# PaddlePaddle/PARL

Measured on NVIDIA H100. Metric: env_steps_per_sec_impala_4096_actors, higher is better.
Workload: dtype bf16 network (fp32 accumulate, fp32 master weights) / f32 scans+losses

## Files before the change

### parl_b200/csrc/shiftconv.cu

```cuda
#include <cuda_bf16.h>

#include "common.cuh"
#include "tma.cuh"
#include "u8win.cuh"
#include "wgmma.cuh"

namespace rl {

constexpr int kScBM = 128;
constexpr int kScMaxStages = 8;
constexpr int kScThreads = 384;

struct ShiftConvArgs {
  const float* bias;
  __nv_bfloat16* out;
  int H, W, KH, KW, Hout, Wout;
  int Q;
  int wrows;
  int num_tiles, relu;
  int stages;
  int out_mode;
  int OGH, OGW;
  int row_shift;
  int flip;
  const __nv_bfloat16* mask;
  float in_scale;
};

__device__ __forceinline__ uint32_t s_pack_bf16x2(float lo, float hi) {
  uint32_t d;
  asm("cvt.rn.bf16x2.f32 %0, %1, %2;\n" : "=r"(d) : "f"(hi), "f"(lo));
  return d;
}
__device__ __forceinline__ uint32_t s_pack_relu_bf16x2(float lo, float hi) {
  uint32_t d;
  asm("cvt.rn.relu.bf16x2.f32 %0, %1, %2;\n" : "=r"(d) : "f"(hi), "f"(lo));
  return d;
}

template <int COUT, int CBLK, int KS, int MODE, bool U8IN = false>
__global__ void __launch_bounds__(U8IN ? kScThreads + kU8Threads : kScThreads, 1)
    shiftconv_fwd_kernel(const __grid_constant__ CUtensorMap map_in, const __grid_constant__ CUtensorMap map_w,
                         const ShiftConvArgs g) {
  static_assert(!U8IN || CBLK == 1, "the uint8 window is one 64-channel block");
  constexpr int W_KB = COUT * 128;
  extern __shared__ __align__(1024) unsigned char smem_dyn[];
  unsigned char* smem = smem_dyn + ((1024u - (smem_u32(smem_dyn) & 1023u)) & 1023u);
  constexpr int num_kb = KS * KS * CBLK;
  const int win_bytes = (g.wrows * 128 + 1023) & ~1023;
  unsigned char* sW = smem;
  unsigned char* sWin = smem + ((num_kb * W_KB + 1023) & ~1023);
  __shared__ __align__(8) unsigned long long full_bar[kScMaxStages], empty_bar[kScMaxStages], w_bar;
  __shared__ __align__(8) unsigned long long u8_full[kU8Stages], u8_empty[kU8Stages];
  const uint32_t nstages = (uint32_t)g.stages;
  unsigned char* sStage = sWin + nstages * CBLK * win_bytes;

  const int warp = threadIdx.x >> 5, lane = threadIdx.x & 31;
  if (threadIdx.x == 0) {
    tma_prefetch_desc(&map_in);
    tma_prefetch_desc(&map_w);
    for (int s = 0; s < kScMaxStages; ++s) {
      mbar_init(&full_bar[s], U8IN ? kU8Threads : 1);
      mbar_init(&empty_bar[s], 1);
    }
    for (int s = 0; s < kU8Stages; ++s) {
      mbar_init(&u8_full[s], 1);
      mbar_init(&u8_empty[s], kU8Threads);
    }
    mbar_init(&w_bar, 1);
    fence_mbar_init();
  }
  __syncthreads();
  if (threadIdx.x == 128) {
    mbar_arrive_expect_tx(&w_bar, (uint32_t)(num_kb * W_KB));
    for (int kb = 0; kb < num_kb; ++kb) tma_load_2d(sW + kb * W_KB, &map_w, kb * 64, 0, &w_bar);
  }
  pdl_wait();
  pdl_trigger();

  if (warp < 4) {
    if (warp == 0 && lane == 0) {
      uint32_t s = 0, par = 1;
      if (U8IN) {
        const int sbytes = u8_stage_bytes(g.wrows);
        for (int tile = blockIdx.x; tile < g.num_tiles; tile += gridDim.x) {
          mbar_wait(&u8_empty[s], par);
          mbar_arrive_expect_tx(&u8_full[s], (uint32_t)(g.wrows * 64));
          tma_load_2d(sStage + s * sbytes, &map_in, 0, tile * kScBM + g.row_shift, &u8_full[s]);
          if (++s == kU8Stages) s = 0, par ^= 1u;
        }
      } else {
        for (int tile = blockIdx.x; tile < g.num_tiles; tile += gridDim.x) {
          mbar_wait(&empty_bar[s], par);
          mbar_arrive_expect_tx(&full_bar[s], (uint32_t)(CBLK * g.wrows * 128));
#pragma unroll
          for (int cb = 0; cb < CBLK; ++cb)
            tma_load_2d(sWin + (s * CBLK + cb) * win_bytes, &map_in, cb * 64, tile * kScBM + g.row_shift, &full_bar[s]);
          if (++s == nstages) s = 0, par ^= 1u;
        }
      }
    }
    return;
  }
  if (U8IN && threadIdx.x >= kScThreads) {
    const int ct = threadIdx.x - kScThreads;
    const int sbytes = u8_stage_bytes(g.wrows);
    const float bias = -8388608.0f * g.in_scale;
    uint32_t s = 0, epar = 1, ss = 0, fpar = 0;
    for (int tile = blockIdx.x; tile < g.num_tiles; tile += gridDim.x) {
      mbar_wait(&u8_full[ss], fpar);
      mbar_wait(&empty_bar[s], epar);
      u8_window_to_bf16_sw128(sStage + ss * sbytes, sWin + s * win_bytes, g.wrows, ct, g.in_scale, bias);
      fence_proxy_async_smem();
      mbar_arrive(&full_bar[s]);
      mbar_arrive(&u8_empty[ss]);
      if (++s == nstages) s = 0, epar ^= 1u;
      if (++ss == kU8Stages) ss = 0, fpar ^= 1u;
    }
    return;
  }
  const int c = (threadIdx.x >> 7) - 1, t = threadIdx.x & 127;
  mbar_wait(&w_bar, 0);
  uint32_t tap_off[KS * KS];
#pragma unroll
  for (int r = 0; r < KS; ++r)
#pragma unroll
    for (int sx = 0; sx < KS; ++sx)
      tap_off[r * KS + sx] = (uint32_t)(g.flip ? (KS - 1 - r) * g.W + (KS - 1 - sx) : r * g.W + sx) * 8u;
  const uint32_t w_lo = gmma_lo(sW), win_lo0 = gmma_lo(sWin);
  const uint32_t win16 = (uint32_t)win_bytes >> 4;
  float bias_r[MODE == 0 ? COUT / 2 : 1];
  if (MODE == 0) {
#pragma unroll
    for (int i = 0; i < COUT / 2; ++i) bias_r[i] = __ldg(g.bias + gmma_col(t, i));
  }
  const bool relu = g.relu != 0;
  const bool has_mask = MODE == 1 && g.mask != nullptr;
  const int HW = g.H * g.W;
  uint32_t s = (uint32_t)c, full_par = 0;
  for (long long tile = blockIdx.x + (long long)c * gridDim.x; tile < g.num_tiles; tile += 2 * gridDim.x) {
    float d[2][COUT / 2];
    mbar_wait(&full_bar[s], full_par);
    wgmma_fence();
    const uint32_t a_lo = win_lo0 + s * (CBLK * win16);
#pragma unroll
    for (int h = 0; h < 2; ++h) {
#pragma unroll
      for (int tap = 0; tap < KS * KS; ++tap) {
#pragma unroll
        for (int cb = 0; cb < CBLK; ++cb) {
#pragma unroll
          for (int k = 0; k < 4; ++k)
            wgmma_bf16<COUT>(d[h], gmma_desc(kGmmaHiSw128, a_lo + h * 512u + cb * win16 + tap_off[tap] + 2u * k),
                             gmma_desc(kGmmaHiSw128, w_lo + (uint32_t)((tap * CBLK + cb) * (W_KB >> 4) + 2 * k)),
                             (tap | cb | k) != 0 ? 1u : 0u);
        }
      }
    }
    wgmma_commit();
    wgmma_wait<0>();
    wgmma_fence_regs(d[0]);
    wgmma_fence_regs(d[1]);
    if (t == 0) mbar_arrive(&empty_bar[s]);
    s += 2;
    if (s >= nstages) s -= nstages, full_par ^= 1u;
#pragma unroll
    for (int h = 0; h < 2; ++h) {
#pragma unroll
      for (int rr = 0; rr < 2; ++rr) {
        const int q = (int)tile * kScBM + 64 * h + gmma_row(t, 2 * rr);
        const int n = q / HW;
        const int rem = q - n * HW;
        const int y = rem / g.W, x = rem - y * g.W;
        const bool valid = q < g.Q && y < g.Hout && x < g.Wout;
        size_t obase = 0;
        if (g.out_mode == 0) {
          obase = ((size_t)(n * g.OGH + y) * g.OGW + x) * COUT;
        } else if (g.out_mode == 1) {
          const int yp = y + 2, xp = x + 2;
          obase = (((size_t)n * 12 + (yp >> 1)) * 12 + (xp >> 1)) * (4 * COUT) + (size_t)(((yp & 1) * 2 + (xp & 1)) * COUT);
        }
        constexpr int MJ = COUT <= 64 ? COUT / 8 : (KS == 2 ? 4 : 2);
#pragma unroll
        for (int j0 = 0; j0 < COUT / 8; j0 += MJ) {
        uint32_t mw[MJ];
        if (has_mask && q < g.Q) {
#pragma unroll
          for (int jj = 0; jj < MJ; ++jj)
            mw[jj] = __ldg(reinterpret_cast<const unsigned int*>(g.mask + (size_t)q * COUT + gmma_col(t, 4 * (j0 + jj) + 2 * rr)));
        }
#pragma unroll
        for (int jj = 0; jj < MJ; ++jj) {
          const int j = j0 + jj, i = 4 * j + 2 * rr, col = gmma_col(t, i);
          bool ok = valid;
          size_t dst_off = obase + col;
          if (g.out_mode == 2) {
            const int blk = col >> 5, py = 2 * y + (blk >> 1) - 2, px = 2 * x + (blk & 1) - 2;
            ok = q < g.Q && py >= 0 && py < 20 && px >= 0 && px < 20;
            dst_off = (((size_t)n * 21 + py) * 21 + px) * 32 + (col & 31);
          }
          if (!ok) continue;
          uint32_t pk;
          if (MODE == 0) {
            const float v0 = d[h][i] + bias_r[i], v1 = d[h][i + 1] + bias_r[i + 1];
            pk = relu ? s_pack_relu_bf16x2(v0, v1) : s_pack_bf16x2(v0, v1);
          } else {
            pk = s_pack_bf16x2(d[h][i], d[h][i + 1]);
            if (has_mask) {
              pk &= __hgt2_mask(*reinterpret_cast<const __nv_bfloat162*>(&mw[jj]), __floats2bfloat162_rn(0.f, 0.f));
            }
          }
          *reinterpret_cast<uint32_t*>(g.out + dst_off) = pk;
        }
        }
      }
    }
  }
}

template <int COUT, int CBLK, int KS, int MODE, bool U8IN = false>
__global__ void __launch_bounds__(U8IN ? kScThreads + kU8Threads : kScThreads, 1)
    shiftconv_coltap_kernel(const __grid_constant__ CUtensorMap map_in, const __grid_constant__ CUtensorMap map_w,
                            const ShiftConvArgs g) {
  static_assert(!U8IN || CBLK == 1, "the uint8 window is one 64-channel block");
  constexpr int W_KB = COUT * 128;
  constexpr int ST = kScBM - (KS - 1);
  extern __shared__ __align__(1024) unsigned char smem_dyn[];
  unsigned char* smem = smem_dyn + ((1024u - (smem_u32(smem_dyn) & 1023u)) & 1023u);
  constexpr int num_kb = KS * KS * CBLK;
  const int win_bytes = (g.wrows * 128 + 1023) & ~1023;
  unsigned char* sW = smem;
  unsigned char* sWin = smem + ((num_kb * W_KB + 1023) & ~1023);
  __shared__ __align__(8) unsigned long long full_bar[kScMaxStages], empty_bar[kScMaxStages], w_bar;
  __shared__ __align__(8) unsigned long long u8_full[kU8Stages], u8_empty[kU8Stages];
  const uint32_t nstages = (uint32_t)g.stages;
  unsigned char* sStage = sWin + nstages * CBLK * win_bytes;
  float* sAcc = reinterpret_cast<float*>(sStage + (U8IN ? kU8Stages * u8_stage_bytes(g.wrows) : 0));

  const int warp = threadIdx.x >> 5, lane = threadIdx.x & 31;
  if (threadIdx.x == 0) {
    tma_prefetch_desc(&map_in);
    tma_prefetch_desc(&map_w);
    for (int s = 0; s < kScMaxStages; ++s) {
      mbar_init(&full_bar[s], U8IN ? kU8Threads : 1);
      mbar_init(&empty_bar[s], 1);
    }
    for (int s = 0; s < kU8Stages; ++s) {
      mbar_init(&u8_full[s], 1);
      mbar_init(&u8_empty[s], kU8Threads);
    }
    mbar_init(&w_bar, 1);
    fence_mbar_init();
  }
  __syncthreads();
  if (threadIdx.x == 128) {
    mbar_arrive_expect_tx(&w_bar, (uint32_t)(num_kb * W_KB));
    for (int kb = 0; kb < num_kb; ++kb) tma_load_2d(sW + kb * W_KB, &map_w, kb * 64, 0, &w_bar);
  }
  pdl_wait();
  pdl_trigger();

  if (warp < 4) {
    if (warp == 0 && lane == 0) {
      uint32_t s = 0, par = 1;
      if (U8IN) {
        const int sbytes = u8_stage_bytes(g.wrows);
        for (int tile = blockIdx.x; tile < g.num_tiles; tile += gridDim.x) {
          mbar_wait(&u8_empty[s], par);
          mbar_arrive_expect_tx(&u8_full[s], (uint32_t)(g.wrows * 64));
          tma_load_2d(sStage + s * sbytes, &map_in, 0, tile * ST + g.row_shift, &u8_full[s]);
          if (++s == kU8Stages) s = 0, par ^= 1u;
        }
      } else {
        for (int tile = blockIdx.x; tile < g.num_tiles; tile += gridDim.x) {
          mbar_wait(&empty_bar[s], par);
          mbar_arrive_expect_tx(&full_bar[s], (uint32_t)(CBLK * g.wrows * 128));
#pragma unroll
          for (int cb = 0; cb < CBLK; ++cb)
            tma_load_2d(sWin + (s * CBLK + cb) * win_bytes, &map_in, cb * 64, tile * ST + g.row_shift, &full_bar[s]);
          if (++s == nstages) s = 0, par ^= 1u;
        }
      }
    }
    return;
  }
  if (U8IN && threadIdx.x >= kScThreads) {
    const int ct = threadIdx.x - kScThreads;
    const int sbytes = u8_stage_bytes(g.wrows);
    const float bias = -8388608.0f * g.in_scale;
    uint32_t s = 0, epar = 1, ss = 0, fpar = 0;
    for (int tile = blockIdx.x; tile < g.num_tiles; tile += gridDim.x) {
      mbar_wait(&u8_full[ss], fpar);
      mbar_wait(&empty_bar[s], epar);
      u8_window_to_bf16_sw128(sStage + ss * sbytes, sWin + s * win_bytes, g.wrows, ct, g.in_scale, bias);
      fence_proxy_async_smem();
      mbar_arrive(&full_bar[s]);
      mbar_arrive(&u8_empty[ss]);
      if (++s == nstages) s = 0, epar ^= 1u;
      if (++ss == kU8Stages) ss = 0, fpar ^= 1u;
    }
    return;
  }
  const int c = (threadIdx.x >> 7) - 1, t = threadIdx.x & 127;
  mbar_wait(&w_bar, 0);
  uint32_t row_off[KS];
#pragma unroll
  for (int r = 0; r < KS; ++r) row_off[r] = (uint32_t)((g.flip ? KS - 1 - r : r) * g.W) * 8u;
  const uint32_t w_lo = gmma_lo(sW), win_lo0 = gmma_lo(sWin);
  const uint32_t win16 = (uint32_t)win_bytes >> 4;
  float bias_r[MODE == 0 ? COUT / 2 : 1];
  if (MODE == 0) {
#pragma unroll
    for (int i = 0; i < COUT / 2; ++i) bias_r[i] = __ldg(g.bias + gmma_col(t, i));
  }
  const bool relu = g.relu != 0;
  const bool has_mask = MODE == 1 && g.mask != nullptr;
  const int HW = g.H * g.W;
  uint32_t s = 0, full_par = 0;
  for (int tile = blockIdx.x; tile < g.num_tiles; tile += gridDim.x) {
    mbar_wait(&full_bar[s], full_par);
    const uint32_t a_lo = win_lo0 + s * (CBLK * win16) + (uint32_t)c * 512u;
#pragma unroll
    for (int sh = 0; sh < KS; ++sh) {
      const int sc = g.flip ? KS - 1 - sh : sh;
      float d[COUT / 2];
      wgmma_fence();
#pragma unroll
      for (int r = 0; r < KS; ++r)
#pragma unroll
        for (int cb = 0; cb < CBLK; ++cb)
#pragma unroll
          for (int k = 0; k < 4; ++k)
            wgmma_bf16<COUT>(d, gmma_desc(kGmmaHiSw128, a_lo + cb * win16 + row_off[r] + 2u * k),
                             gmma_desc(kGmmaHiSw128, w_lo + (uint32_t)(((r * KS + sc) * CBLK + cb) * (W_KB >> 4) + 2 * k)),
                             (r | cb | k) != 0 ? 1u : 0u);
      wgmma_commit();
      wgmma_wait<0>();
      wgmma_fence_regs(d);
      named_bar_sync(1, 256);
      if (sh == KS - 1 && threadIdx.x == 128) mbar_arrive(&empty_bar[s]);
#pragma unroll
      for (int i = 0; i < COUT / 2; i += 2) {
        const int p = 64 * c + gmma_row(t, i) - sh;
        if (p < 0) continue;
        float2* cell = reinterpret_cast<float2*>(sAcc + p * COUT + gmma_col(t, i));
        if (sh == 0) {
          *cell = make_float2(d[i], d[i + 1]);
        } else {
          const float2 o = *cell;
          *cell = make_float2(o.x + d[i], o.y + d[i + 1]);
        }
      }
    }
    if (++s == nstages) s = 0, full_par ^= 1u;
    named_bar_sync(1, 256);
#pragma unroll
    for (int i = 0; i < COUT / 2; i += 2) {
      const int p = 64 * c + gmma_row(t, i), col = gmma_col(t, i);
      const int q = tile * ST + p;
      if (p >= ST || q >= g.Q) continue;
      const float2 v = *reinterpret_cast<const float2*>(sAcc + p * COUT + col);
      const int n = q / HW;
      const int rem = q - n * HW;
      const int y = rem / g.W, x = rem - y * g.W;
      bool ok = y < g.Hout && x < g.Wout;
      size_t dst_off;
      if (g.out_mode == 0) {
        dst_off = ((size_t)(n * g.OGH + y) * g.OGW + x) * COUT + col;
      } else if (g.out_mode == 1) {
        const int yp = y + 2, xp = x + 2;
        dst_off = (((size_t)n * 12 + (yp >> 1)) * 12 + (xp >> 1)) * (4 * COUT) + (size_t)(((yp & 1) * 2 + (xp & 1)) * COUT) + col;
      } else {
        const int blk = col >> 5, py = 2 * y + (blk >> 1) - 2, px = 2 * x + (blk & 1) - 2;
        ok = py >= 0 && py < 20 && px >= 0 && px < 20;
        dst_off = (((size_t)n * 21 + py) * 21 + px) * 32 + (col & 31);
      }
      if (!ok) continue;
      uint32_t pk;
      if (MODE == 0) {
        const float v0 = v.x + bias_r[i], v1 = v.y + bias_r[i + 1];
        pk = relu ? s_pack_relu_bf16x2(v0, v1) : s_pack_bf16x2(v0, v1);
      } else {
        pk = s_pack_bf16x2(v.x, v.y);
        if (has_mask) {
          const uint32_t mw = __ldg(reinterpret_cast<const unsigned int*>(g.mask + (size_t)q * COUT + col));
          pk &= __hgt2_mask(*reinterpret_cast<const __nv_bfloat162*>(&mw), __floats2bfloat162_rn(0.f, 0.f));
        }
      }
      *reinterpret_cast<uint32_t*>(g.out + dst_off) = pk;
    }
  }
}

static int sc_make_map(CUtensorMap* map, const void* base, uint64_t cols, uint64_t rows, uint32_t box_rows) {
  typedef CUresult (*EncodeFn)(CUtensorMap*, CUtensorMapDataType, cuuint32_t, void*, const cuuint64_t*, const cuuint64_t*,
                               const cuuint32_t*, const cuuint32_t*, CUtensorMapInterleave, CUtensorMapSwizzle,
                               CUtensorMapL2promotion, CUtensorMapFloatOOBfill);
  static EncodeFn fn = nullptr;
  if (!fn) {
    void* p = nullptr;
    cudaDriverEntryPointQueryResult q;
    if (cudaGetDriverEntryPoint("cuTensorMapEncodeTiled", &p, cudaEnableDefault, &q) != cudaSuccess || !p) return -1;
    fn = reinterpret_cast<EncodeFn>(p);
  }
  const cuuint64_t gdim[2] = {cols, rows};
  const cuuint64_t gstride[1] = {cols * 2};
  const cuuint32_t box[2] = {64, box_rows};
  const cuuint32_t estr[2] = {1, 1};
  return fn(map, CU_TENSOR_MAP_DATA_TYPE_BFLOAT16, 2, const_cast<void*>(base), gdim, gstride, box, estr,
            CU_TENSOR_MAP_INTERLEAVE_NONE, CU_TENSOR_MAP_SWIZZLE_128B, CU_TENSOR_MAP_L2_PROMOTION_L2_128B,
            CU_TENSOR_MAP_FLOAT_OOB_FILL_NONE) == CUDA_SUCCESS
             ? 0
             : -2;
}

static size_t u8_ring_bytes(int wrows) { return (size_t)kU8Stages * (size_t)((wrows * 64 + 1023) & ~1023); }

template <int COUT, int CBLK, int KS, int MODE, bool U8IN = false>
static void launch_shiftconv(const CUtensorMap& mi, const CUtensorMap& mw, const ShiftConvArgs& g, int num_kb, int sms,
                             cudaStream_t st) {
  const size_t win = (size_t)((g.wrows * 128 + 1023) & ~1023);
  const size_t smem = (size_t)((num_kb * COUT * 128 + 1023) & ~1023) + (size_t)g.stages * CBLK * win + 1024 +
                      (U8IN ? u8_ring_bytes(g.wrows) : 0);
  auto kern = shiftconv_fwd_kernel<COUT, CBLK, KS, MODE, U8IN>;
  RL_SMEM_OPTIN(kern);
  const int grid = g.num_tiles < sms ? g.num_tiles : sms;
  launch_chain(kern, dim3(grid), dim3(U8IN ? kScThreads + kU8Threads : kScThreads), smem, st, mi, mw, g);
}

template <int COUT, int CBLK, int KS, int MODE, bool U8IN = false>
static void launch_coltap(const CUtensorMap& mi, const CUtensorMap& mw, const ShiftConvArgs& g, int num_kb, int sms,
                          cudaStream_t st) {
  const size_t win = (size_t)((g.wrows * 128 + 1023) & ~1023);
  const size_t smem = (size_t)((num_kb * COUT * 128 + 1023) & ~1023) + (size_t)g.stages * CBLK * win + 1024 +
                      (U8IN ? u8_ring_bytes(g.wrows) : 0) + (size_t)kScBM * COUT * sizeof(float);
  auto kern = shiftconv_coltap_kernel<COUT, CBLK, KS, MODE, U8IN>;
  RL_SMEM_OPTIN(kern);
  const int grid = g.num_tiles < sms ? g.num_tiles : sms;
  launch_chain(kern, dim3(grid), dim3(U8IN ? kScThreads + kU8Threads : kScThreads), smem, st, mi, mw, g);
}

}

using namespace rl;

static int g_sc_form = 0;
extern "C" int rl_debug_set_shiftconv_form(int form) {
  RL_CHECK_ARG(form == 0 || form == 1, "shiftconv form must be 0 (per-tap) or 1 (column taps)");
  g_sc_form = form;
  return RL_OK;
}

extern "C" int rl_debug_set_shiftconv_base_offset(int enable) {
  RL_CHECK_ARG(enable == 0, "shiftconv base_offset must be 0 (the swizzle phase comes from the shared-memory address)");
  return RL_OK;
}

static int shiftconv_launch(const void* in, const void* weight, const float* bias, void* out, int N, int H, int W,
                            int Cin, int Cout, int KH, int KW, int relu, int out_mode, int Hout, int Wout, int OGH, int OGW,
                            int transposed, const void* mask, rl_stream_t stream, const char* name, int u8in = 0,
                            float in_scale = 1.f) {
  RL_CHECK_ARG(in && weight && out && N > 0, "%s: bad argument", name);
  RL_CHECK_ARG(aligned16(in) && aligned16(weight) && aligned16(out) && (!mask || aligned16(mask)),
               "%s: 16-byte alignment required", name);
  RL_CHECK_ARG((Cout == 32 || Cout == 64 || Cout == 128) && (Cin == 64 || Cin == 128),
               "%s: Cin in {64,128}, Cout in {32,64,128}", name);
  RL_CHECK_ARG(KH == KW && (KH == 2 || KH == 3) && KH <= H && KW <= W, "%s: filter must be 2x2 or 3x3", name);
  ShiftConvArgs g;
  g.bias = bias, g.out = (__nv_bfloat16*)out, g.H = H, g.W = W, g.KH = KH, g.KW = KW;
  g.Hout = Hout, g.Wout = Wout, g.OGH = OGH, g.OGW = OGW;
  const long long Q = (long long)N * H * W;
  RL_CHECK_ARG(Q < (1LL << 31), "%s: too many positions", name);
  const int coltap = g_sc_form == 1;
  const int tile_rows = coltap ? kScBM - (KW - 1) : kScBM;
  g.Q = (int)Q, g.wrows = kScBM + (KH - 1) * W + (coltap ? 0 : KW - 1), g.relu = relu, g.out_mode = out_mode;
  g.row_shift = transposed ? -((KH - 1) * W + (KW - 1)) : 0, g.flip = transposed;
  g.mask = (const __nv_bfloat16*)mask, g.in_scale = in_scale;
  RL_CHECK_ARG(g.wrows <= 256, "%s: window of %d rows exceeds the TMA box limit", name, g.wrows);
  g.num_tiles = (int)((Q + tile_rows - 1) / tile_rows);
  const int cblk = Cin / 64, num_kb = KH * KW * cblk;
  const size_t win = (size_t)((g.wrows * 128 + 1023) & ~1023);
  {
    const size_t acc = coltap ? (size_t)kScBM * Cout * sizeof(float) : 0;
    const size_t budget = 220 * 1024 - ((size_t)num_kb * Cout * 128 + 2048) - (u8in ? u8_ring_bytes(g.wrows) : 0) - acc;
    long long st = (long long)(budget / ((size_t)cblk * win));
    if (st > kScMaxStages) st = kScMaxStages;
    if (mask && st > 4) st = 4;
    RL_CHECK_ARG(st >= 2, "%s: weights + windows do not fit in shared memory", name);
    g.stages = (int)st;
  }
  alignas(64) CUtensorMap mi, mw;
  if ((u8in ? make_tensor_map_u8_rows64(&mi, in, (uint64_t)Q, (uint32_t)g.wrows)
            : sc_make_map(&mi, in, (uint64_t)Cin, (uint64_t)Q, (uint32_t)g.wrows)) ||
      sc_make_map(&mw, weight, (uint64_t)KH * KW * Cin, (uint64_t)Cout, (uint32_t)Cout)) {
    set_error("%s: cuTensorMapEncodeTiled failed", name);
    return RL_ERR_CUDA;
  }
  int dev = 0, sms = 132;
  cudaGetDevice(&dev);
  cudaDeviceGetAttribute(&sms, cudaDevAttrMultiProcessorCount, dev);
  sms = effective_sms(sms);
  cudaStream_t st = (cudaStream_t)stream;
  const int key = (u8in ? 1000000 : 0) + (transposed ? 100000 : 0) + Cout * 100 + cblk * 10 + KH;
  if (coltap) {
    switch (key) {
      case 1003212: launch_coltap<32, 1, 2, 0, true>(mi, mw, g, num_kb, sms, st); break;
      case 3212: launch_coltap<32, 1, 2, 0>(mi, mw, g, num_kb, sms, st); break;
      case 6422: launch_coltap<64, 2, 2, 0>(mi, mw, g, num_kb, sms, st); break;
      case 6413: launch_coltap<64, 1, 3, 0>(mi, mw, g, num_kb, sms, st); break;
      case 6412: launch_coltap<64, 1, 2, 0>(mi, mw, g, num_kb, sms, st); break;
      case 6423: launch_coltap<64, 2, 3, 0>(mi, mw, g, num_kb, sms, st); break;
      case 106413: launch_coltap<64, 1, 3, 1>(mi, mw, g, num_kb, sms, st); break;
      case 112812: launch_coltap<128, 1, 2, 1>(mi, mw, g, num_kb, sms, st); break;
      case 106412: launch_coltap<64, 1, 2, 1>(mi, mw, g, num_kb, sms, st); break;
      case 112813: launch_coltap<128, 1, 3, 1>(mi, mw, g, num_kb, sms, st); break;
      default:
        set_error("%s: no instantiation for Cout=%d Cin=%d %dx%d", name, Cout, Cin, KH, KW);
        return RL_ERR_BAD_ARG;
    }
  } else
  switch (key) {
    case 1003212: launch_shiftconv<32, 1, 2, 0, true>(mi, mw, g, num_kb, sms, st); break;
    case 3212: launch_shiftconv<32, 1, 2, 0>(mi, mw, g, num_kb, sms, st); break;
    case 6422: launch_shiftconv<64, 2, 2, 0>(mi, mw, g, num_kb, sms, st); break;
    case 6413: launch_shiftconv<64, 1, 3, 0>(mi, mw, g, num_kb, sms, st); break;
    case 6412: launch_shiftconv<64, 1, 2, 0>(mi, mw, g, num_kb, sms, st); break;
    case 6423: launch_shiftconv<64, 2, 3, 0>(mi, mw, g, num_kb, sms, st); break;
    case 106413: launch_shiftconv<64, 1, 3, 1>(mi, mw, g, num_kb, sms, st); break;
    case 112812: launch_shiftconv<128, 1, 2, 1>(mi, mw, g, num_kb, sms, st); break;
    case 106412: launch_shiftconv<64, 1, 2, 1>(mi, mw, g, num_kb, sms, st); break;
    case 112813: launch_shiftconv<128, 1, 3, 1>(mi, mw, g, num_kb, sms, st); break;
    default:
      set_error("%s: no instantiation for Cout=%d Cin=%d %dx%d", name, Cout, Cin, KH, KW);
      return RL_ERR_BAD_ARG;
  }
  cudaError_t e = cudaGetLastError();
  if (e != cudaSuccess) {
    set_error("%s: launch failed: %s", name, cudaGetErrorString(e));
    return RL_ERR_CUDA;
  }
  return RL_OK;
}

extern "C" int rl_conv2d_s1_nhwc_bf16_fwd(const void* in, const void* weight_krsc, const float* bias, void* out, int N,
                                          int H, int W, int Cin, int Cout, int KH, int KW, int relu, int out_mode,
                                          rl_stream_t stream) {
  RL_CHECK_ARG(bias, "conv2d_s1: bias required");
  RL_CHECK_ARG(out_mode == 0 || (out_mode == 1 && H - KH + 1 == 20 && W - KW + 1 == 20),
               "conv2d_s1: out_mode 1 is the 20x20 -> [12,12,4*Cout] layout");
  return shiftconv_launch(in, weight_krsc, bias, out, N, H, W, Cin, Cout, KH, KW, relu, out_mode, H - KH + 1, W - KW + 1,
                          H - KH + 1, W - KW + 1, 0, nullptr, stream, "conv2d_s1");
}

extern "C" int rl_conv2d_s1_u8in_bf16_fwd(const void* in_u8, float in_scale, const void* weight_krsc, const float* bias,
                                          void* out, int N, int H, int W, int Cout, int KH, int KW, int relu,
                                          int out_mode, rl_stream_t stream) {
  RL_CHECK_ARG(bias, "conv2d_s1_u8in: bias required");
  RL_CHECK_ARG(Cout == 32 && KH == 2 && KW == 2, "conv2d_s1_u8in: built for the 2x2, 64 -> 32 layer (conv1, space-to-depth)");
  RL_CHECK_ARG(out_mode == 0 || (out_mode == 1 && H - KH + 1 == 20 && W - KW + 1 == 20),
               "conv2d_s1_u8in: out_mode 1 is the 20x20 -> [12,12,4*Cout] layout");
  return shiftconv_launch(in_u8, weight_krsc, bias, out, N, H, W, 64, Cout, KH, KW, relu, out_mode, H - KH + 1,
                          W - KW + 1, H - KH + 1, W - KW + 1, 0, nullptr, stream, "conv2d_s1_u8in", 1, in_scale);
}

extern "C" int rl_conv2d_s1_nhwc_bf16_dgrad(const void* dout_grid, const void* weight_t_krsc, const void* act_mask,
                                            void* din, int N, int H, int W, int Cout, int Cin, int KH, int KW,
                                            int out_mode, int OGH, int OGW, rl_stream_t stream) {
  RL_CHECK_ARG(out_mode == 0 || (out_mode == 2 && H == 12 && W == 12 && Cin == 128),
               "conv2d_s1_dgrad: out_mode 2 is the [12,12,128] -> [21,21,32] layout");
  return shiftconv_launch(dout_grid, weight_t_krsc, nullptr, din, N, H, W, Cout, Cin, KH, KW, 0, out_mode, H, W,
                          out_mode == 0 ? OGH : 0, out_mode == 0 ? OGW : 0, 1, act_mask, stream, "conv2d_s1_dgrad");
}
```

### parl_b200/csrc/wgmma.cuh

```cuda
#pragma once
#include <stdint.h>

#include "tma.cuh"

namespace rl {

#ifdef __CUDACC__
constexpr uint32_t kGmmaHiSw128 = (uint32_t)(1024 >> 4) | (1u << 30);
constexpr uint32_t kGmmaHiSw64 = (uint32_t)(512 >> 4) | (2u << 30);
constexpr uint32_t kGmmaLoLbo1 = 1u << 16;
__device__ __forceinline__ uint64_t gmma_desc(uint32_t hi, uint32_t lo) { return ((uint64_t)hi << 32) | (uint64_t)lo; }
__device__ __forceinline__ uint32_t gmma_lo(const void* smem) { return (smem_u32(smem) >> 4) + kGmmaLoLbo1; }

__device__ __forceinline__ void wgmma_fence() { asm volatile("wgmma.fence.sync.aligned;\n" ::: "memory"); }
__device__ __forceinline__ void wgmma_commit() { asm volatile("wgmma.commit_group.sync.aligned;\n" ::: "memory"); }
template <int N>
__device__ __forceinline__ void wgmma_wait() {
  asm volatile("wgmma.wait_group.sync.aligned %0;\n" ::"n"(N) : "memory");
}
template <int R>
__device__ __forceinline__ void wgmma_fence_regs(float (&d)[R]) {
#pragma unroll
  for (int i = 0; i < R; ++i) asm volatile("" : "+f"(d[i])::"memory");
}
__device__ __forceinline__ void named_bar_sync(int id, int nthreads) {
  asm volatile("bar.sync %0, %1;\n" ::"r"(id), "r"(nthreads) : "memory");
}

template <int TA, int TB>
__device__ __forceinline__ void wgmma_bf16_n32(float (&d)[16], uint64_t da, uint64_t db, uint32_t acc) {
  asm volatile(
      "{\n.reg .pred p;\nsetp.ne.b32 p, %18, 0;\n"
      "wgmma.mma_async.sync.aligned.m64n32k16.f32.bf16.bf16 {%0, %1, %2, %3, %4, %5, %6, %7, %8, %9, %10, %11, %12, %13, %14, %15}, %16, %17, p, 1, 1, %19, %20;\n}\n"
      : "+f"(d[0]), "+f"(d[1]), "+f"(d[2]), "+f"(d[3]), "+f"(d[4]), "+f"(d[5]), "+f"(d[6]), "+f"(d[7]), "+f"(d[8]), "+f"(d[9]), "+f"(d[10]), "+f"(d[11]), "+f"(d[12]), "+f"(d[13]), "+f"(d[14]), "+f"(d[15])
      : "l"(da), "l"(db), "r"(acc), "n"(TA), "n"(TB));
}
template <int TA, int TB>
__device__ __forceinline__ void wgmma_bf16_n64(float (&d)[32], uint64_t da, uint64_t db, uint32_t acc) {
  asm volatile(
      "{\n.reg .pred p;\nsetp.ne.b32 p, %34, 0;\n"
      "wgmma.mma_async.sync.aligned.m64n64k16.f32.bf16.bf16 {%0, %1, %2, %3, %4, %5, %6, %7, %8, %9, %10, %11, %12, %13, %14, %15, %16, %17, %18, %19, %20, %21, %22, %23, %24, %25, %26, %27, %28, %29, %30, %31}, %32, %33, p, 1, 1, %35, %36;\n}\n"
      : "+f"(d[0]), "+f"(d[1]), "+f"(d[2]), "+f"(d[3]), "+f"(d[4]), "+f"(d[5]), "+f"(d[6]), "+f"(d[7]), "+f"(d[8]), "+f"(d[9]), "+f"(d[10]), "+f"(d[11]), "+f"(d[12]), "+f"(d[13]), "+f"(d[14]), "+f"(d[15]), "+f"(d[16]), "+f"(d[17]), "+f"(d[18]), "+f"(d[19]), "+f"(d[20]), "+f"(d[21]), "+f"(d[22]), "+f"(d[23]), "+f"(d[24]), "+f"(d[25]), "+f"(d[26]), "+f"(d[27]), "+f"(d[28]), "+f"(d[29]), "+f"(d[30]), "+f"(d[31])
      : "l"(da), "l"(db), "r"(acc), "n"(TA), "n"(TB));
}
template <int TA, int TB>
__device__ __forceinline__ void wgmma_bf16_n128(float (&d)[64], uint64_t da, uint64_t db, uint32_t acc) {
  asm volatile(
      "{\n.reg .pred p;\nsetp.ne.b32 p, %66, 0;\n"
      "wgmma.mma_async.sync.aligned.m64n128k16.f32.bf16.bf16 {%0, %1, %2, %3, %4, %5, %6, %7, %8, %9, %10, %11, %12, %13, %14, %15, %16, %17, %18, %19, %20, %21, %22, %23, %24, %25, %26, %27, %28, %29, %30, %31, %32, %33, %34, %35, %36, %37, %38, %39, %40, %41, %42, %43, %44, %45, %46, %47, %48, %49, %50, %51, %52, %53, %54, %55, %56, %57, %58, %59, %60, %61, %62, %63}, %64, %65, p, 1, 1, %67, %68;\n}\n"
      : "+f"(d[0]), "+f"(d[1]), "+f"(d[2]), "+f"(d[3]), "+f"(d[4]), "+f"(d[5]), "+f"(d[6]), "+f"(d[7]), "+f"(d[8]), "+f"(d[9]), "+f"(d[10]), "+f"(d[11]), "+f"(d[12]), "+f"(d[13]), "+f"(d[14]), "+f"(d[15]), "+f"(d[16]), "+f"(d[17]), "+f"(d[18]), "+f"(d[19]), "+f"(d[20]), "+f"(d[21]), "+f"(d[22]), "+f"(d[23]), "+f"(d[24]), "+f"(d[25]), "+f"(d[26]), "+f"(d[27]), "+f"(d[28]), "+f"(d[29]), "+f"(d[30]), "+f"(d[31]), "+f"(d[32]), "+f"(d[33]), "+f"(d[34]), "+f"(d[35]), "+f"(d[36]), "+f"(d[37]), "+f"(d[38]), "+f"(d[39]), "+f"(d[40]), "+f"(d[41]), "+f"(d[42]), "+f"(d[43]), "+f"(d[44]), "+f"(d[45]), "+f"(d[46]), "+f"(d[47]), "+f"(d[48]), "+f"(d[49]), "+f"(d[50]), "+f"(d[51]), "+f"(d[52]), "+f"(d[53]), "+f"(d[54]), "+f"(d[55]), "+f"(d[56]), "+f"(d[57]), "+f"(d[58]), "+f"(d[59]), "+f"(d[60]), "+f"(d[61]), "+f"(d[62]), "+f"(d[63])
      : "l"(da), "l"(db), "r"(acc), "n"(TA), "n"(TB));
}
template <int TA, int TB>
__device__ __forceinline__ void wgmma_bf16_n256(float (&d)[128], uint64_t da, uint64_t db, uint32_t acc) {
  asm volatile(
      "{\n.reg .pred p;\nsetp.ne.b32 p, %130, 0;\n"
      "wgmma.mma_async.sync.aligned.m64n256k16.f32.bf16.bf16 {%0, %1, %2, %3, %4, %5, %6, %7, %8, %9, %10, %11, %12, %13, %14, %15, %16, %17, %18, %19, %20, %21, %22, %23, %24, %25, %26, %27, %28, %29, %30, %31, %32, %33, %34, %35, %36, %37, %38, %39, %40, %41, %42, %43, %44, %45, %46, %47, %48, %49, %50, %51, %52, %53, %54, %55, %56, %57, %58, %59, %60, %61, %62, %63, %64, %65, %66, %67, %68, %69, %70, %71, %72, %73, %74, %75, %76, %77, %78, %79, %80, %81, %82, %83, %84, %85, %86, %87, %88, %89, %90, %91, %92, %93, %94, %95, %96, %97, %98, %99, %100, %101, %102, %103, %104, %105, %106, %107, %108, %109, %110, %111, %112, %113, %114, %115, %116, %117, %118, %119, %120, %121, %122, %123, %124, %125, %126, %127}, %128, %129, p, 1, 1, %131, %132;\n}\n"
      : "+f"(d[0]), "+f"(d[1]), "+f"(d[2]), "+f"(d[3]), "+f"(d[4]), "+f"(d[5]), "+f"(d[6]), "+f"(d[7]), "+f"(d[8]), "+f"(d[9]), "+f"(d[10]), "+f"(d[11]), "+f"(d[12]), "+f"(d[13]), "+f"(d[14]), "+f"(d[15]), "+f"(d[16]), "+f"(d[17]), "+f"(d[18]), "+f"(d[19]), "+f"(d[20]), "+f"(d[21]), "+f"(d[22]), "+f"(d[23]), "+f"(d[24]), "+f"(d[25]), "+f"(d[26]), "+f"(d[27]), "+f"(d[28]), "+f"(d[29]), "+f"(d[30]), "+f"(d[31]), "+f"(d[32]), "+f"(d[33]), "+f"(d[34]), "+f"(d[35]), "+f"(d[36]), "+f"(d[37]), "+f"(d[38]), "+f"(d[39]), "+f"(d[40]), "+f"(d[41]), "+f"(d[42]), "+f"(d[43]), "+f"(d[44]), "+f"(d[45]), "+f"(d[46]), "+f"(d[47]), "+f"(d[48]), "+f"(d[49]), "+f"(d[50]), "+f"(d[51]), "+f"(d[52]), "+f"(d[53]), "+f"(d[54]), "+f"(d[55]), "+f"(d[56]), "+f"(d[57]), "+f"(d[58]), "+f"(d[59]), "+f"(d[60]), "+f"(d[61]), "+f"(d[62]), "+f"(d[63]), "+f"(d[64]), "+f"(d[65]), "+f"(d[66]), "+f"(d[67]), "+f"(d[68]), "+f"(d[69]), "+f"(d[70]), "+f"(d[71]), "+f"(d[72]), "+f"(d[73]), "+f"(d[74]), "+f"(d[75]), "+f"(d[76]), "+f"(d[77]), "+f"(d[78]), "+f"(d[79]), "+f"(d[80]), "+f"(d[81]), "+f"(d[82]), "+f"(d[83]), "+f"(d[84]), "+f"(d[85]), "+f"(d[86]), "+f"(d[87]), "+f"(d[88]), "+f"(d[89]), "+f"(d[90]), "+f"(d[91]), "+f"(d[92]), "+f"(d[93]), "+f"(d[94]), "+f"(d[95]), "+f"(d[96]), "+f"(d[97]), "+f"(d[98]), "+f"(d[99]), "+f"(d[100]), "+f"(d[101]), "+f"(d[102]), "+f"(d[103]), "+f"(d[104]), "+f"(d[105]), "+f"(d[106]), "+f"(d[107]), "+f"(d[108]), "+f"(d[109]), "+f"(d[110]), "+f"(d[111]), "+f"(d[112]), "+f"(d[113]), "+f"(d[114]), "+f"(d[115]), "+f"(d[116]), "+f"(d[117]), "+f"(d[118]), "+f"(d[119]), "+f"(d[120]), "+f"(d[121]), "+f"(d[122]), "+f"(d[123]), "+f"(d[124]), "+f"(d[125]), "+f"(d[126]), "+f"(d[127])
      : "l"(da), "l"(db), "r"(acc), "n"(TA), "n"(TB));
}
template <int N, int TA = 0, int TB = 0>
__device__ __forceinline__ void wgmma_bf16(float (&d)[N / 2], uint64_t da, uint64_t db, uint32_t acc) {
  static_assert(N == 32 || N == 64 || N == 128 || N == 256, "wgmma_bf16: N in {32, 64, 128, 256}");
  if constexpr (N == 32) wgmma_bf16_n32<TA, TB>(d, da, db, acc);
  else if constexpr (N == 64) wgmma_bf16_n64<TA, TB>(d, da, db, acc);
  else if constexpr (N == 128) wgmma_bf16_n128<TA, TB>(d, da, db, acc);
  else wgmma_bf16_n256<TA, TB>(d, da, db, acc);
}

__device__ __forceinline__ int gmma_row(int t, int i) { return 16 * (t >> 5) + ((t & 31) >> 2) + 8 * ((i >> 1) & 1); }
__device__ __forceinline__ int gmma_col(int t, int i) { return 8 * (i >> 2) + 2 * (t & 3) + (i & 1); }
#endif

}
```

Measured before the change: 2.915 million.

## Stage shiftconv data-gradient epilogue through swizzled smem with TMA-loaded mask

For the transposed (MODE 1) shift-conv, the ReLU mask is now fetched by the TMA producer into a per-stage swizzled smem tile alongside the input window. The accumulators are masked via ldmatrix/stmatrix in smem, and each thread then writes 16-byte rows to global memory instead of scattered 4-byte stores and per-thread mask __ldg. The goal is coalesced output stores and mask reads that overlap with the GEMM pipeline. In exchange, the stage ring holds an extra output tile per stage (the old cap of 4 stages when a mask is present is removed), the empty barrier now needs 128 arrivals, and the epilogue adds a named barrier.

New measurement: 3.247 million (median of 6 runs). +11.4%, better.

```diff
diff --git a/parl_b200/csrc/shiftconv.cu b/parl_b200/csrc/shiftconv.cu
--- a/parl_b200/csrc/shiftconv.cu
+++ b/parl_b200/csrc/shiftconv.cu
@@ -10,6 +10,7 @@
 constexpr int kScBM = 128;
 constexpr int kScMaxStages = 8;
 constexpr int kScThreads = 384;
+constexpr int kScEpiBar = 1;
 
 struct ShiftConvArgs {
   const float* bias;
@@ -38,12 +39,18 @@
   return d;
 }
 
+__device__ __forceinline__ uint32_t sc_tile_off(int row, int ch) {
+  return (uint32_t)((ch >> 3) * (kScBM * 128) + row * 128 + (((ch & 7) ^ (row & 7)) << 4));
+}
+
 template <int COUT, int CBLK, int KS, int MODE, bool U8IN = false>
 __global__ void __launch_bounds__(U8IN ? kScThreads + kU8Threads : kScThreads, 1)
     shiftconv_fwd_kernel(const __grid_constant__ CUtensorMap map_in, const __grid_constant__ CUtensorMap map_w,
-                         const ShiftConvArgs g) {
+                         const __grid_constant__ CUtensorMap map_mask, const ShiftConvArgs g) {
   static_assert(!U8IN || CBLK == 1, "the uint8 window is one 64-channel block");
+  static_assert(MODE == 0 || COUT % 64 == 0, "the data gradient's tile is made of 64-column mask boxes");
   constexpr int W_KB = COUT * 128;
+  constexpr int OUT_BYTES = kScBM * COUT * 2;
   extern __shared__ __align__(1024) unsigned char smem_dyn[];
   unsigned char* smem = smem_dyn + ((1024u - (smem_u32(smem_dyn) & 1023u)) & 1023u);
   constexpr int num_kb = KS * KS * CBLK;
@@ -54,14 +61,17 @@
   __shared__ __align__(8) unsigned long long u8_full[kU8Stages], u8_empty[kU8Stages];
   const uint32_t nstages = (uint32_t)g.stages;
   unsigned char* sStage = sWin + nstages * CBLK * win_bytes;
+  unsigned char* sOut = sWin + nstages * CBLK * win_bytes;
+  const bool has_mask = MODE == 1 && g.mask != nullptr;
 
   const int warp = threadIdx.x >> 5, lane = threadIdx.x & 31;
   if (threadIdx.x == 0) {
     tma_prefetch_desc(&map_in);
     tma_prefetch_desc(&map_w);
+    if (has_mask) tma_prefetch_desc(&map_mask);
     for (int s = 0; s < kScMaxStages; ++s) {
       mbar_init(&full_bar[s], U8IN ? kU8Threads : 1);
-      mbar_init(&empty_bar[s], 1);
+      mbar_init(&empty_bar[s], MODE == 0 ? 1 : 128);
     }
     for (int s = 0; s < kU8Stages; ++s) {
       mbar_init(&u8_full[s], 1);
@@ -90,12 +100,18 @@
           if (++s == kU8Stages) s = 0, par ^= 1u;
         }
       } else {
+        const uint32_t tx = (uint32_t)(CBLK * g.wrows * 128) + (has_mask ? (uint32_t)OUT_BYTES : 0u);
         for (int tile = blockIdx.x; tile < g.num_tiles; tile += gridDim.x) {
           mbar_wait(&empty_bar[s], par);
-          mbar_arrive_expect_tx(&full_bar[s], (uint32_t)(CBLK * g.wrows * 128));
+          mbar_arrive_expect_tx(&full_bar[s], tx);
 #pragma unroll
           for (int cb = 0; cb < CBLK; ++cb)
             tma_load_2d(sWin + (s * CBLK + cb) * win_bytes, &map_in, cb * 64, tile * kScBM + g.row_shift, &full_bar[s]);
+          if (has_mask) {
+#pragma unroll
+            for (int cb = 0; cb < COUT / 64; ++cb)
+              tma_load_2d(sOut + s * OUT_BYTES + cb * (kScBM * 128), &map_mask, cb * 64, tile * kScBM, &full_bar[s]);
+          }
           if (++s == nstages) s = 0, par ^= 1u;
         }
       }
@@ -135,8 +151,11 @@
     for (int i = 0; i < COUT / 2; ++i) bias_r[i] = __ldg(g.bias + gmma_col(t, i));
   }
   const bool relu = g.relu != 0;
-  const bool has_mask = MODE == 1 && g.mask != nullptr;
   const int HW = g.H * g.W;
+  constexpr int CH = COUT / 8;
+  const int mx_row = 16 * (t >> 5) + (lane & 7) + 8 * ((lane >> 3) & 1), mx_ch = lane >> 4;
+  constexpr int RSTEP = kScBM / CH;
+  const int cp_ch = t % CH, cp_row = t / CH;
   uint32_t s = (uint32_t)c, full_par = 0;
   for (long long tile = blockIdx.x + (long long)c * gridDim.x; tile < g.num_tiles; tile += 2 * gridDim.x) {
     float d[2][COUT / 2];
@@ -161,58 +180,86 @@
     wgmma_wait<0>();
     wgmma_fence_regs(d[0]);
     wgmma_fence_regs(d[1]);
-    if (t == 0) mbar_arrive(&empty_bar[s]);
-    s += 2;
-    if (s >= nstages) s -= nstages, full_par ^= 1u;
-#pragma unroll
-    for (int h = 0; h < 2; ++h) {
-#pragma unroll
-      for (int rr = 0; rr < 2; ++rr) {
-        const int q = (int)tile * kScBM + 64 * h + gmma_row(t, 2 * rr);
-        const int n = q / HW;
-        const int rem = q - n * HW;
-        const int y = rem / g.W, x = rem - y * g.W;
-        const bool valid = q < g.Q && y < g.Hout && x < g.Wout;
-        size_t obase = 0;
+    if constexpr (MODE == 0) {
+      if (t == 0) mbar_arrive(&empty_bar[s]);
+      s += 2;
+      if (s >= nstages) s -= nstages, full_par ^= 1u;
+#pragma unroll
+      for (int h = 0; h < 2; ++h) {
+#pragma unroll
+        for (int rr = 0; rr < 2; ++rr) {
+          const int q = (int)tile * kScBM + 64 * h + gmma_row(t, 2 * rr);
+          const int n = q / HW;
+          const int rem = q - n * HW;
+          const int y = rem / g.W, x = rem - y * g.W;
+          const bool valid = q < g.Q && y < g.Hout && x < g.Wout;
+          size_t obase;
+          if (g.out_mode == 0) {
+            obase = ((size_t)(n * g.OGH + y) * g.OGW + x) * COUT;
+          } else {
+            const int yp = y + 2, xp = x + 2;
+            obase = (((size_t)n * 12 + (yp >> 1)) * 12 + (xp >> 1)) * (4 * COUT) + (size_t)(((yp & 1) * 2 + (xp & 1)) * COUT);
+          }
+#pragma unroll
+          for (int j = 0; j < CH; ++j) {
+            const int i = 4 * j + 2 * rr;
+            if (!valid) continue;
+            const float v0 = d[h][i] + bias_r[i], v1 = d[h][i + 1] + bias_r[i + 1];
+            *reinterpret_cast<uint32_t*>(g.out + obase + gmma_col(t, i)) =
+                relu ? s_pack_relu_bf16x2(v0, v1) : s_pack_bf16x2(v0, v1);
+          }
+        }
+      }
+    } else {
+      const unsigned char* tile_p = sOut + s * OUT_BYTES;
+      const uint32_t otile = smem_u32(tile_p);
+#pragma unroll
+      for (int h = 0; h < 2; ++h) {
+#pragma unroll
+        for (int j = 0; j < CH; j += 2) {
+          uint32_t pk[4];
+#pragma unroll
+          for (int m = 0; m < 4; ++m) pk[m] = s_pack_bf16x2(d[h][4 * j + 2 * m], d[h][4 * j + 2 * m + 1]);
+          const uint32_t a = otile + sc_tile_off(64 * h + mx_row, j + mx_ch);
+          if (has_mask) {
+            uint32_t mw[4];
+            ldmatrix_x4(a, mw);
+#pragma unroll
+            for (int m = 0; m < 4; ++m)
+              pk[m] &= __hgt2_mask(*reinterpret_cast<const __nv_bfloat162*>(&mw[m]), __floats2bfloat162_rn(0.f, 0.f));
+          }
+          stmatrix_x4(a, pk);
+        }
+      }
+      named_bar_sync(kScEpiBar + c, 128);
+      uint4 v[CH];
+#pragma unroll
+      for (int k = 0; k < CH; ++k) v[k] = *reinterpret_cast<const uint4*>(tile_p + sc_tile_off(cp_row + RSTEP * k, cp_ch));
+      fence_proxy_async_smem();
+      mbar_arrive(&empty_bar[s]);
+      s += 2;
+      if (s >= nstages) s -= nstages, full_par ^= 1u;
+      int q = (int)tile * kScBM + cp_row;
+      int n = q / HW;
+      int y = (q - n * HW) / g.W;
+      int x = q - n * HW - y * g.W;
+#pragma unroll
+      for (int k = 0; k < CH; ++k) {
+        const int col = 8 * cp_ch;
+        bool ok = q < g.Q;
+        size_t dst_off;
         if (g.out_mode == 0) {
-          obase = ((size_t)(n * g.OGH + y) * g.OGW + x) * COUT;
-        } else if (g.out_mode == 1) {
-          const int yp = y + 2, xp = x + 2;
-          obase = (((size_t)n * 12 + (yp >> 1)) * 12 + (xp >> 1)) * (4 * COUT) + (size_t)(((yp & 1) * 2 + (xp & 1)) * COUT);
-        }
-        constexpr int MJ = COUT <= 64 ? COUT / 8 : (KS == 2 ? 4 : 2);
-#pragma unroll
-        for (int j0 = 0; j0 < COUT / 8; j0 += MJ) {
-        uint32_t mw[MJ];
-        if (has_mask && q < g.Q) {
-#pragma unroll
-          for (int jj = 0; jj < MJ; ++jj)
-            mw[jj] = __ldg(reinterpret_cast<const unsigned int*>(g.mask + (size_t)q * COUT + gmma_col(t, 4 * (j0 + jj) + 2 * rr)));
-        }
-#pragma unroll
-        for (int jj = 0; jj < MJ; ++jj) {
-          const int j = j0 + jj, i = 4 * j + 2 * rr, col = gmma_col(t, i);
-          bool ok = valid;
-          size_t dst_off = obase + col;
-          if (g.out_mode == 2) {
-            const int blk = col >> 5, py = 2 * y + (blk >> 1) - 2, px = 2 * x + (blk & 1) - 2;
-            ok = q < g.Q && py >= 0 && py < 20 && px >= 0 && px < 20;
-            dst_off = (((size_t)n * 21 + py) * 21 + px) * 32 + (col & 31);
-          }
-          if (!ok) continue;
-          uint32_t pk;
-          if (MODE == 0) {
-            const float v0 = d[h][i] + bias_r[i], v1 = d[h][i + 1] + bias_r[i + 1];
-            pk = relu ? s_pack_relu_bf16x2(v0, v1) : s_pack_bf16x2(v0, v1);
-          } else {
-            pk = s_pack_bf16x2(d[h][i], d[h][i + 1]);
-            if (has_mask) {
-              pk &= __hgt2_mask(*reinterpret_cast<const __nv_bfloat162*>(&mw[jj]), __floats2bfloat162_rn(0.f, 0.f));
-            }
-          }
-          *reinterpret_cast<uint32_t*>(g.out + dst_off) = pk;
-        }
-        }
+          ok = ok && y < g.Hout && x < g.Wout;
+          dst_off = ((size_t)(n * g.OGH + y) * g.OGW + x) * COUT + col;
+        } else {
+          const int blk = col >> 5, py = 2 * y + (blk >> 1) - 2, px = 2 * x + (blk & 1) - 2;
+          ok = ok && py >= 0 && py < 20 && px >= 0 && px < 20;
+          dst_off = (((size_t)n * 21 + py) * 21 + px) * 32 + (col & 31);
+        }
+        if (ok) *reinterpret_cast<uint4*>(g.out + dst_off) = v[k];
+        q += RSTEP;
+        for (x += RSTEP; x >= g.W; x -= g.W)
+          if (++y == g.H) y = 0, ++n;
       }
     }
   }
@@ -417,15 +464,16 @@
 static size_t u8_ring_bytes(int wrows) { return (size_t)kU8Stages * (size_t)((wrows * 64 + 1023) & ~1023); }
 
 template <int COUT, int CBLK, int KS, int MODE, bool U8IN = false>
-static void launch_shiftconv(const CUtensorMap& mi, const CUtensorMap& mw, const ShiftConvArgs& g, int num_kb, int sms,
-                             cudaStream_t st) {
+static void launch_shiftconv(const CUtensorMap& mi, const CUtensorMap& mw, const CUtensorMap& mm, const ShiftConvArgs& g,
+                             int num_kb, int sms, cudaStream_t st) {
   const size_t win = (size_t)((g.wrows * 128 + 1023) & ~1023);
-  const size_t smem = (size_t)((num_kb * COUT * 128 + 1023) & ~1023) + (size_t)g.stages * CBLK * win + 1024 +
+  const size_t tile = MODE == 1 ? (size_t)kScBM * COUT * 2 : 0;
+  const size_t smem = (size_t)((num_kb * COUT * 128 + 1023) & ~1023) + (size_t)g.stages * (CBLK * win + tile) + 1024 +
                       (U8IN ? u8_ring_bytes(g.wrows) : 0);
   auto kern = shiftconv_fwd_kernel<COUT, CBLK, KS, MODE, U8IN>;
   RL_SMEM_OPTIN(kern);
   const int grid = g.num_tiles < sms ? g.num_tiles : sms;
-  launch_chain(kern, dim3(grid), dim3(U8IN ? kScThreads + kU8Threads : kScThreads), smem, st, mi, mw, g);
+  launch_chain(kern, dim3(grid), dim3(U8IN ? kScThreads + kU8Threads : kScThreads), smem, st, mi, mw, mm, g);
 }
 
 template <int COUT, int CBLK, int KS, int MODE, bool U8IN = false>
@@ -482,20 +530,22 @@
   const size_t win = (size_t)((g.wrows * 128 + 1023) & ~1023);
   {
     const size_t acc = coltap ? (size_t)kScBM * Cout * sizeof(float) : 0;
+    const size_t tile = transposed && !coltap ? (size_t)kScBM * Cout * 2 : 0;
     const size_t budget = 220 * 1024 - ((size_t)num_kb * Cout * 128 + 2048) - (u8in ? u8_ring_bytes(g.wrows) : 0) - acc;
-    long long st = (long long)(budget / ((size_t)cblk * win));
+    long long st = (long long)(budget / ((size_t)cblk * win + tile));
     if (st > kScMaxStages) st = kScMaxStages;
-    if (mask && st > 4) st = 4;
     RL_CHECK_ARG(st >= 2, "%s: weights + windows do not fit in shared memory", name);
     g.stages = (int)st;
   }
-  alignas(64) CUtensorMap mi, mw;
+  alignas(64) CUtensorMap mi, mw, mm;
   if ((u8in ? make_tensor_map_u8_rows64(&mi, in, (uint64_t)Q, (uint32_t)g.wrows)
             : sc_make_map(&mi, in, (uint64_t)Cin, (uint64_t)Q, (uint32_t)g.wrows)) ||
-      sc_make_map(&mw, weight, (uint64_t)KH * KW * Cin, (uint64_t)Cout, (uint32_t)Cout)) {
+      sc_make_map(&mw, weight, (uint64_t)KH * KW * Cin, (uint64_t)Cout, (uint32_t)Cout) ||
+      (mask && !coltap && sc_make_map(&mm, mask, (uint64_t)Cout, (uint64_t)Q, (uint32_t)kScBM))) {
     set_error("%s: cuTensorMapEncodeTiled failed", name);
     return RL_ERR_CUDA;
   }
+  if (!mask || coltap) mm = mi;
   int dev = 0, sms = 132;
   cudaGetDevice(&dev);
   cudaDeviceGetAttribute(&sms, cudaDevAttrMultiProcessorCount, dev);
@@ -520,16 +570,16 @@
     }
   } else
   switch (key) {
-    case 1003212: launch_shiftconv<32, 1, 2, 0, true>(mi, mw, g, num_kb, sms, st); break;
-    case 3212: launch_shiftconv<32, 1, 2, 0>(mi, mw, g, num_kb, sms, st); break;
-    case 6422: launch_shiftconv<64, 2, 2, 0>(mi, mw, g, num_kb, sms, st); break;
-    case 6413: launch_shiftconv<64, 1, 3, 0>(mi, mw, g, num_kb, sms, st); break;
-    case 6412: launch_shiftconv<64, 1, 2, 0>(mi, mw, g, num_kb, sms, st); break;
-    case 6423: launch_shiftconv<64, 2, 3, 0>(mi, mw, g, num_kb, sms, st); break;
-    case 106413: launch_shiftconv<64, 1, 3, 1>(mi, mw, g, num_kb, sms, st); break;
-    case 112812: launch_shiftconv<128, 1, 2, 1>(mi, mw, g, num_kb, sms, st); break;
-    case 106412: launch_shiftconv<64, 1, 2, 1>(mi, mw, g, num_kb, sms, st); break;
-    case 112813: launch_shiftconv<128, 1, 3, 1>(mi, mw, g, num_kb, sms, st); break;
+    case 1003212: launch_shiftconv<32, 1, 2, 0, true>(mi, mw, mm, g, num_kb, sms, st); break;
+    case 3212: launch_shiftconv<32, 1, 2, 0>(mi, mw, mm, g, num_kb, sms, st); break;
+    case 6422: launch_shiftconv<64, 2, 2, 0>(mi, mw, mm, g, num_kb, sms, st); break;
+    case 6413: launch_shiftconv<64, 1, 3, 0>(mi, mw, mm, g, num_kb, sms, st); break;
+    case 6412: launch_shiftconv<64, 1, 2, 0>(mi, mw, mm, g, num_kb, sms, st); break;
+    case 6423: launch_shiftconv<64, 2, 3, 0>(mi, mw, mm, g, num_kb, sms, st); break;
+    case 106413: launch_shiftconv<64, 1, 3, 1>(mi, mw, mm, g, num_kb, sms, st); break;
+    case 112812: launch_shiftconv<128, 1, 2, 1>(mi, mw, mm, g, num_kb, sms, st); break;
+    case 106412: launch_shiftconv<64, 1, 2, 1>(mi, mw, mm, g, num_kb, sms, st); break;
+    case 112813: launch_shiftconv<128, 1, 3, 1>(mi, mw, mm, g, num_kb, sms, st); break;
     default:
       set_error("%s: no instantiation for Cout=%d Cin=%d %dx%d", name, Cout, Cin, KH, KW);
       return RL_ERR_BAD_ARG;
diff --git a/parl_b200/csrc/wgmma.cuh b/parl_b200/csrc/wgmma.cuh
--- a/parl_b200/csrc/wgmma.cuh
+++ b/parl_b200/csrc/wgmma.cuh
@@ -70,6 +70,18 @@
 
 __device__ __forceinline__ int gmma_row(int t, int i) { return 16 * (t >> 5) + ((t & 31) >> 2) + 8 * ((i >> 1) & 1); }
 __device__ __forceinline__ int gmma_col(int t, int i) { return 8 * (i >> 2) + 2 * (t & 3) + (i & 1); }
+
+__device__ __forceinline__ void ldmatrix_x4(uint32_t addr, uint32_t (&r)[4]) {
+  asm volatile("ldmatrix.sync.aligned.m8n8.x4.shared.b16 {%0, %1, %2, %3}, [%4];\n"
+               : "=r"(r[0]), "=r"(r[1]), "=r"(r[2]), "=r"(r[3])
+               : "r"(addr)
+               : "memory");
+}
+__device__ __forceinline__ void stmatrix_x4(uint32_t addr, const uint32_t (&r)[4]) {
+  asm volatile("stmatrix.sync.aligned.m8n8.x4.shared.b16 [%0], {%1, %2, %3, %4};\n" ::"r"(addr), "r"(r[0]), "r"(r[1]),
+               "r"(r[2]), "r"(r[3])
+               : "memory");
+}
 #endif
 
 }
```
